# henriChevreux/distillation_trajectories

Hardware: AMD Instinct MI355X
Metric: trajectory-timesteps/sec (B×T U-Net fwd) at 16×16 T=50 (higher is better)
Workload: dtype f32 (fp32-accurate; convolutions: exact 3-plane bf16 operand split on bf16 MFMA with fp32 accumulate, or native fp32 MFMA, chosen per layer)

## Files before the change

distillation_trajectories_amd/csrc/build.py:

```python
import os
import shutil
import subprocess
import sys

HERE = os.path.dirname(os.path.abspath(__file__))
SOURCES = ["dt_conv.hip", "dt_conv_bf16.hip", "dt_conv_strip.hip", "dt_layers.hip", "dt_update.hip", "dt_metrics.hip", "dt_fused.hip", "dt_unet.hip",
           "dt_featnet.hip", "dt_inception.hip", "dt_pca.hip", "dt_fid.hip", "dt_lpips.hip", "dt_tsne.hip", "dt_quality.hip", "dt_quality_stream.hip", "dt_edit.hip", "dt_rng.hip"]
HEADERS = ["dt_internal.h", "dt_conv_forms.h", "dt_batch.h", "dt_dense64.h", "dt_quality_math.h", "dt_featnet.h", "dt_conv_epilogue.h", "dt_conv_walk.h", "dt_update_math.h", "dt_fused.h", os.path.join("..", "..", "include", "dt_hip.h"),
           os.path.join("..", "..", "include", "dt_hip_noise.h"),
           os.path.join("..", "..", "include", "dt_hip_inception.h"),
           os.path.join("..", "..", "include", "dt_hip_pca.h"),
           os.path.join("..", "..", "include", "dt_hip_fid.h"),
           os.path.join("..", "..", "include", "dt_hip_fid_cov.h"),
           os.path.join("..", "..", "include", "dt_hip_lpips.h"),
           os.path.join("..", "..", "include", "dt_hip_tsne.h"),
           os.path.join("..", "..", "include", "dt_hip_quality.h"),
           os.path.join("..", "..", "include", "dt_hip_quality_stream.h"),
           os.path.join("..", "..", "include", "dt_hip_edit.h"),
           os.path.join("..", "..", "include", "dt_hip_rng.h")]
LIB = os.path.join(HERE, "libdt_hip.so")
ARCH = "gfx950"


def hipcc_path():
    for cand in (os.environ.get("HIPCC"), "/opt/rocm/bin/hipcc", shutil.which("hipcc")):
        if cand and os.path.exists(cand):
            return cand
    raise RuntimeError("hipcc not found (looked at $HIPCC, /opt/rocm/bin/hipcc, PATH)")


OBJ_DIR = os.path.join(HERE, "_build")
# ... 113 lines not shown
```

distillation_trajectories_amd/csrc/dt_conv.hip:

```cpp
#include "dt_conv_walk.h"

namespace dt {

template <int BM, int BN>
__global__ __launch_bounds__(256, 4) void conv_gemm_kernel(const ConvParams p) {
  constexpr ConvForm F = *find_conv_form(KIND_FP32, BM, BN);
  constexpr int WN = F.wn();
  constexpr int MI = F.mi(), NI = F.ni();
  constexpr int A_PER = BM / 64, B_PER = BN / 64;
  constexpr int STAGE = (BM + BN) * 16;
  constexpr int LDS_FLOATS = 2 * STAGE > F.stage_floats() ? 2 * STAGE : F.stage_floats();
  static_assert(F.wm() == 2 && WN == 2 && MI * 64 == BM && NI * 64 == BN && LDS_FLOATS >= F.stage_floats(), "wave layout, epilogue stage");
  __shared__ __attribute__((aligned(16))) float lds[LDS_FLOATS];

  const int tid = threadIdx.x, lane = tid & 63, wave = tid >> 6;
  const int wm = wave / WN, wn = wave % WN;
  const int half = lane >> 5, l31 = lane & 31;
  const int m0 = blockIdx.x * BM, n0 = blockIdx.y * BN;
  const int HW = p.H * p.W;

  int a_off[A_PER], a_off2[A_PER], a_y[A_PER], a_x[A_PER];
  bool a_ok[A_PER];
  int a_lds[A_PER];
#pragma unroll
  for (int j = 0; j < A_PER; ++j) {
    const int q = tid + j * 256, row = q >> 2, pslot = q & 3;
    const int lslot = pslot ^ ((row >> 2) & 3);
    const int m = m0 + row;
    a_ok[j] = m < p.M;
    const int mm = a_ok[j] ? m : 0;
    const int b = mm / HW, rem = mm - b * HW;
    a_y[j] = rem / p.W;
    a_x[j] = rem - a_y[j] * p.W;
    a_off[j] = mm * p.cin_p + lslot * 4;
    a_off2[j] = mm * p.cin2_p + lslot * 4;
    a_lds[j] = q * 4;
  }
  const float *wbase = p.w + (size_t)n0 * 16 + tid * 4;

  f32x16 acc[MI][NI];
  DT_CLEAR_ACC(acc, MI, NI);

  int a_row[MI], b_row[NI];
#pragma unroll
  for (int mi = 0; mi < MI; ++mi) a_row[mi] = wm * (MI * 32) + mi * 32 + l31;
#pragma unroll
  for (int ni = 0; ni < NI; ++ni) b_row[ni] = wn * (NI * 32) + ni * 32 + l31;

  KWalk k(p);
  const int n_main = k.n_main, n_iter = k.n_iter;
  for (int it = -1; it < n_iter; ++it) {
    const bool more = it + 1 < n_iter;
    f32x4 ra[A_PER], rb[B_PER];
    if (more && it + 1 >= n_main) {
      const int c2 = it + 1 - n_main;
#pragma unroll
// ... 29 lines not shown
#pragma unroll
        for (int ni = 0; ni < NI; ++ni)
          fb[ni] = *reinterpret_cast<const f32x4 *>(B + b_row[ni] * 16 + (((2 * s + half) ^ ((b_row[ni] >> 2) & 3)) << 2));
#pragma unroll
        for (int i = 0; i < 4; ++i)
#pragma unroll
          for (int mi = 0; mi < MI; ++mi)
#pragma unroll
            for (int ni = 0; ni < NI; ++ni) {
              acc[mi][ni] = __builtin_amdgcn_mfma_f32_32x32x2f32(fa[mi][i], fb[ni][i], acc[mi][ni], 0, 0, 0);
            }
      }
    }
    if (more) {
      float *A = lds + ((it + 1) & 1) * STAGE, *B = A + BM * 16;
#pragma unroll
      for (int j = 0; j < A_PER; ++j) *reinterpret_cast<f32x4 *>(A + a_lds[j]) = ra[j];
#pragma unroll
      for (int j = 0; j < B_PER; ++j) *reinterpret_cast<f32x4 *>(B + (tid + j * 256) * 4) = rb[j];
    }
    __syncthreads();
  }

  conv_epilogue<BM, BN, 1>(p, acc, lds, m0, n0, wm, wn, half, l31);
}

int launch_splitk_epilogue(const ConvParams &p, hipStream_t s);

#define DT_GEMM_ROW(cls, kind, bm, bn, kc, wk) {{kind, bm, bn, kc, wk, cls}, conv_gemm_kernel<bm, bn>},
static const ConvKernel kGemmKernels[] = {DT_CONV_FORMS_FP32(DT_GEMM_ROW)};

int launch_conv(const ConvParams &p, hipStream_t s) {
  if (!p.in || !p.w || !p.scale || !p.shift || !p.out) return DT_E_NULL;
  if (p.cin_p % 16 || p.cout_p % 16 || p.n_p % kNPad || p.M <= 0) return DT_E_SHAPE;
  if ((long long)p.M * p.cin_p >= (1ll << 31) || (long long)p.M * p.cout_p * (p.n_dup > 1 ? p.n_dup : 1) >= (1ll << 31)) return DT_E_SHAPE;
  if (const int st = conv_admissible(p)) return st;
  {
    const double flops = 2.0 * p.M * (double)p.cout_real * ((double)p.cin_real * p.ksize * p.ksize + (p.in2 ? p.cin2_real : 0));
    ProfileScope prof(find_conv_form(p.kind, p.bm, p.bn)->cls, flops, 4.0 * p.M * ((double)p.cin_real + p.cout_real), s);
    if (p.kind == KIND_FP32) {
      conv_kernel_of(kGemmKernels, p).fn<<<dim3((p.M + p.bm - 1) / p.bm, p.n_p / p.bn, p.splits), 256, 0, s>>>(p);
      DT_LAUNCH_CHECK();
    } else if (const int st = is_strip(p.kind) ? launch_conv_strip(p, s) : launch_conv_bf16x6(p, s)) return st;
  }
  return p.splits > 1 ? launch_splitk_epilogue(p, s) : DT_OK;
}


bool conv_choice_valid(const ConvChoice &c, int slot, int n_p) {
  if (!find_conv_form(c.kind, c.bm, c.bn) || n_p % c.bn) return false;
  if (c.splits < 1 || c.splits > 9 || c.splits == 5 || c.splits == 6 || c.splits == 7) return false;
  return !c.fuse || (slot == 2 && c.splits == 1);
}

static ConvChoice heuristic_choice(int M, int n_p, int taps) {
  ConvChoice c{};
// ... 44 lines not shown

template <int S>
__device__ inline float4 splitk_finish(const ConvParams &p, unsigned m, int n, size_t slab_stride) {
  const size_t o = (size_t)m * p.cout_p + n;
  float4 a;
  if (S > 0) {
    float4 part[S > 0 ? S : 1];
#pragma unroll
    for (int z = 0; z < S; ++z) part[z] = *reinterpret_cast<const float4 *>(p.slab + z * slab_stride + o);
    a = part[0];
#pragma unroll
    for (int z = 1; z < S; ++z) { a.x += part[z].x; a.y += part[z].y; a.z += part[z].z; a.w += part[z].w; }
  } else {
    a = *reinterpret_cast<const float4 *>(p.slab + o);
    for (int z = 1; z < p.splits; ++z) {
      const float4 b = *reinterpret_cast<const float4 *>(p.slab + z * slab_stride + o);
      a.x += b.x; a.y += b.y; a.z += b.z; a.w += b.w;
    }
  }
  const float4 sc = *reinterpret_cast<const float4 *>(p.scale + n), sh = *reinterpret_cast<const float4 *>(p.shift + n);
  float4 v = make_float4(a.x * sc.x + sh.x, a.y * sc.y + sh.y, a.z * sc.z + sh.z, a.w * sc.w + sh.w);
  if (p.relu) { v.x = fmaxf(v.x, 0.f); v.y = fmaxf(v.y, 0.f); v.z = fmaxf(v.z, 0.f); v.w = fmaxf(v.w, 0.f); }
  if (p.tb) {
    const float4 t = *reinterpret_cast<const float4 *>(p.tb + (size_t)(m / (unsigned)p.m_per_tb) * p.tb_stride + n);
    v.x += t.x; v.y += t.y; v.z += t.z; v.w += t.w;
  }
  if (p.add) {
    const float4 t = *reinterpret_cast<const float4 *>(p.add + o);
    v.x += t.x; v.y += t.y; v.z += t.z; v.w += t.w;
  }
  *reinterpret_cast<float4 *>(p.out + o) = v;
  return v;
}

template <int S, bool POOL>
__global__ __launch_bounds__(256) void splitk_epilogue_kernel(const ConvParams p) {
  const unsigned c4 = (unsigned)p.cout_p >> 2;
  const size_t slab_stride = (size_t)p.M * p.cout_p;
  if (!POOL) {
    const unsigned total = (unsigned)p.M * c4;
    const bool pow2 = (c4 & (c4 - 1)) == 0;
    const int sh4 = 31 - __builtin_clz(c4);
    for (unsigned i = blockIdx.x * blockDim.x + threadIdx.x; i < total; i += gridDim.x * blockDim.x) {
      const unsigned m = pow2 ? i >> sh4 : i / c4;
      splitk_finish<S>(p, m, (int)(i - m * c4) * 4, slab_stride);
    }
  } else {
    const unsigned Wo = (unsigned)p.W >> 1, Ho = (unsigned)p.H >> 1, HW = (unsigned)(p.H * p.W);
    const unsigned total = ((unsigned)p.M >> 2) * c4;
    for (unsigned i = blockIdx.x * blockDim.x + threadIdx.x; i < total; i += gridDim.x * blockDim.x) {
      const unsigned wq = i / c4;
      const int n = (int)(i - wq * c4) * 4;
      const unsigned xo = wq % Wo, r = wq / Wo;
      const unsigned yo = r % Ho, b = r / Ho;
      const unsigned m00 = b * HW + 2 * yo * (unsigned)p.W + 2 * xo;
      const float4 a = splitk_finish<S>(p, m00, n, slab_stride), bq = splitk_finish<S>(p, m00 + 1, n, slab_stride);
      const float4 c = splitk_finish<S>(p, m00 + p.W, n, slab_stride), d = splitk_finish<S>(p, m00 + p.W + 1, n, slab_stride);
      float4 mx;
      mx.x = fmaxf(fmaxf(a.x, bq.x), fmaxf(c.x, d.x)); mx.y = fmaxf(fmaxf(a.y, bq.y), fmaxf(c.y, d.y));
      mx.z = fmaxf(fmaxf(a.z, bq.z), fmaxf(c.z, d.z)); mx.w = fmaxf(fmaxf(a.w, bq.w), fmaxf(c.w, d.w));
      *reinterpret_cast<float4 *>(p.pool_out + (size_t)wq * p.cout_p + n) = mx;
    }
  }
}

template <bool POOL>
static int launch_splitk_epilogue_t(const ConvParams &p, hipStream_t s) {
  const size_t total = (size_t)(POOL ? p.M / 4 : p.M) * (p.cout_p / 4);
  const int blocks = grid_blocks(total, 4096);
  ProfileScope prof(KC_SPLITK_EPILOGUE, 0.0, 4.0 * p.M * p.cout_p * (p.splits + 1.0 + (POOL ? 0.25 : 0.0)), s);
  switch (p.splits) {
    case 2: splitk_epilogue_kernel<2, POOL><<<blocks, 256, 0, s>>>(p); break;
    case 3: splitk_epilogue_kernel<3, POOL><<<blocks, 256, 0, s>>>(p); break;
    case 4: splitk_epilogue_kernel<4, POOL><<<blocks, 256, 0, s>>>(p); break;
    case 8: splitk_epilogue_kernel<8, POOL><<<blocks, 256, 0, s>>>(p); break;
    case 9: splitk_epilogue_kernel<9, POOL><<<blocks, 256, 0, s>>>(p); break;
    default: splitk_epilogue_kernel<0, POOL><<<blocks, 256, 0, s>>>(p); break;
  }
// ... 82 lines not shown
```

distillation_trajectories_amd/csrc/dt_conv_bf16.hip:

```cpp
#include "dt_conv_walk.h"

namespace dt {

template <int BM, int BN>
__global__ __launch_bounds__(256, BM * BN > 128 * 128 ? 2 : 3) void conv_gemm_bf16x6_kernel(const ConvParams p) {
  constexpr ConvForm F = *find_conv_form(KIND_BF16, BM, BN);
  constexpr int WM = F.wm(), WN = F.wn();
  constexpr int MI = F.mi(), NI = F.ni();
  static_assert(WM == 2 && WN == 2 && MI * 64 == BM && NI * 64 == BN, "wave layout");
  constexpr int PLANE_A = BM * 16, PLANE_B = BN * 16;
  constexpr int STAGE = 3 * (PLANE_A + PLANE_B);
  __shared__ __attribute__((aligned(16))) __bf16 lds[2 * STAGE];

  const int tid = threadIdx.x, lane = tid & 63, wave = tid >> 6;
  const int wm = wave / WN, wn = wave % WN;
  const int half = lane >> 5, l31 = lane & 31;
  const int m0 = blockIdx.x * BM, n0 = blockIdx.y * BN;
  const int HW = p.H * p.W;

  constexpr int NT = 64 * WM * WN;
  constexpr int AP = (BM * 2 + NT - 1) / NT, BP = (BN * 2 + NT - 1) / NT;
  bool a_ok[AP];
  int a_y[AP], a_x[AP], a_off[AP], a_off2[AP], a_lds[AP];
#pragma unroll
  for (int i = 0; i < AP; ++i) {
    const int item = tid + i * NT;
    const int rowi = item >> 1, hh = item & 1;
    const int m = m0 + rowi;
    a_ok[i] = item < BM * 2 && m < p.M;
    const int mm = a_ok[i] ? m : 0;
    const int b = mm / HW, rem = mm - b * HW;
    a_y[i] = rem / p.W; a_x[i] = rem - a_y[i] * p.W;
    a_off[i] = mm * p.cin_p + hh * 8;
    a_off2[i] = mm * p.cin2_p + hh * 8;
    a_lds[i] = rowi * 16 + ((hh ^ ((rowi >> 3) & 1)) << 3);
  }
  const __bf16 *wbase = reinterpret_cast<const __bf16 *>(p.w) + (size_t)n0 * 16 + tid * 8;
  const size_t w_plane = (size_t)p.n_p * 16;

  f32x16 acc[MI][NI];
  DT_CLEAR_ACC(acc, MI, NI);

  int a_frag[MI], b_frag[NI];
#pragma unroll
  for (int mi = 0; mi < MI; ++mi) {
    const int row = wm * (MI * 32) + mi * 32 + l31;
    a_frag[mi] = row * 16 + ((half ^ ((row >> 3) & 1)) << 3);
  }
#pragma unroll
  for (int ni = 0; ni < NI; ++ni) {
    const int row = wn * (NI * 32) + ni * 32 + l31;
    b_frag[ni] = row * 16 + ((half ^ ((row >> 3) & 1)) << 3);
  }

  KWalk k(p);
// ... 61 lines not shown
      }
    }
    if (more) {
      __bf16 *A = lds + ((it + 1) & 1) * STAGE, *B = A + 3 * PLANE_A;
#pragma unroll
      for (int i = 0; i < AP; ++i)
        if (tid + i * NT < BM * 2) {
          bf16x8 p1, p2, p3;
          split8(ra0[i], ra1[i], p1, p2, p3);
          *reinterpret_cast<bf16x8 *>(A + a_lds[i]) = p1;
          *reinterpret_cast<bf16x8 *>(A + PLANE_A + a_lds[i]) = p2;
          *reinterpret_cast<bf16x8 *>(A + 2 * PLANE_A + a_lds[i]) = p3;
        }
#pragma unroll
      for (int i = 0; i < BP; ++i)
        if (tid + i * NT < BN * 2) {
#pragma unroll
          for (int pl = 0; pl < 3; ++pl) *reinterpret_cast<u32x4 *>(B + pl * PLANE_B + (tid + i * NT) * 8) = rb[i][pl];
        }
    }
    __syncthreads();
  }
  static_assert(2 * STAGE * sizeof(__bf16) >= F.stage_bytes(), "epilogue stage");
  conv_epilogue<BM, BN, 1>(p, acc, reinterpret_cast<float *>(lds), m0, n0, wm, wn, half, l31);
}

#define DT_BF16_ROW(cls, kind, bm, bn, kc, wk) {{kind, bm, bn, kc, wk, cls}, conv_gemm_bf16x6_kernel<bm, bn>},
static const ConvKernel kBf16Kernels[] = {DT_CONV_FORMS_BF16(DT_BF16_ROW)};

int launch_conv_bf16x6(const ConvParams &p, hipStream_t s) {
  conv_kernel_of(kBf16Kernels, p).fn<<<dim3((p.M + p.bm - 1) / p.bm, p.n_p / p.bn, p.splits), 256, 0, s>>>(p);
  DT_LAUNCH_CHECK();
  return DT_OK;
}

__global__ void pack_conv_bf16x3_kernel(const float *__restrict__ w, __bf16 *__restrict__ wp, int cout, int cin,
                                        int ksize, int cin_p, int cin_w, int n_p, int split_c, int split_cp, size_t total) {
  for (size_t idx = blockIdx.x * (size_t)blockDim.x + threadIdx.x; idx < total; idx += (size_t)gridDim.x * blockDim.x) {
    const int pos = idx & 15;
    const size_t rowi = idx >> 4;
    const int n = rowi % n_p;
    const size_t kc = rowi / n_p;
    const int phh = pos >> 3, j = pos & 7;
    const int hh = phh ^ ((n >> 3) & 1);
    const int k = (int)kc * 16 + hh * 8 + j;
    const int tap = k / cin_w, cp = k - tap * cin_w;
    const int c = conv_real_channel(cp, cin, cin_p, split_c, split_cp);
// ... 25 lines not shown
```

distillation_trajectories_amd/csrc/dt_conv_epilogue.h:

```cpp
#pragma once
#include "dt_internal.h"

namespace dt {

typedef float f32x16 __attribute__((ext_vector_type(16)));
typedef float f32x4 __attribute__((ext_vector_type(4)));

typedef __bf16 bf16x8 __attribute__((ext_vector_type(8)));
typedef __bf16 bf16x2 __attribute__((ext_vector_type(2)));
typedef unsigned u32x4 __attribute__((ext_vector_type(4)));

__device__ inline float bf16_to_f32(__bf16 v) { return (float)v; }

__device__ inline void split8(const f32x4 lo, const f32x4 hi, bf16x8 &p1, bf16x8 &p2, bf16x8 &p3) {
#pragma unroll
  for (int i = 0; i < 8; ++i) {
    const float a = i < 4 ? lo[i] : hi[i - 4];
    const __bf16 a1 = (__bf16)a;
    const float r1 = a - (float)a1;
    const __bf16 a2 = (__bf16)r1;
    const float r2 = r1 - (float)a2;
    p1[i] = a1; p2[i] = a2; p3[i] = (__bf16)r2;
  }
}

__device__ inline void mfma_bf16x6(f32x16 &acc, const bf16x8 (&fa)[3], const bf16x8 (&fb)[3]) {
  f32x16 c = acc;
  c = __builtin_amdgcn_mfma_f32_32x32x16_bf16(fa[2], fb[0], c, 0, 0, 0);
  c = __builtin_amdgcn_mfma_f32_32x32x16_bf16(fa[1], fb[1], c, 0, 0, 0);
  c = __builtin_amdgcn_mfma_f32_32x32x16_bf16(fa[0], fb[2], c, 0, 0, 0);
  c = __builtin_amdgcn_mfma_f32_32x32x16_bf16(fa[1], fb[0], c, 0, 0, 0);
  c = __builtin_amdgcn_mfma_f32_32x32x16_bf16(fa[0], fb[1], c, 0, 0, 0);
  c = __builtin_amdgcn_mfma_f32_32x32x16_bf16(fa[0], fb[0], c, 0, 0, 0);
  acc = c;
}

template <int BM, int BN, int WK, int MI, int NI>
__device__ inline void conv_epilogue(const ConvParams &p, f32x16 (&acc)[MI][NI], float *stage, int m0, int n0, int wm, int wn,
                                     int half, int l31, int wk = 0) {
  constexpr ConvForm F = *find_conv_layout(BM, BN, WK);
  static_assert(MI == F.mi() && NI == F.ni(), "accumulator tiles of the form");
  constexpr int WM = F.wm(), P = F.pitch(), C4 = BN / 4, U = WM * C4 / 8;
  constexpr int COPY = F.copy_floats();
  const int tid = threadIdx.x;
  const int HW = p.H * p.W;
  const bool pow2 = (p.W & (p.W - 1)) == 0 && (HW & (HW - 1)) == 0;
  const int w_sh = 31 - __builtin_clz(p.W), hw_sh = 31 - __builtin_clz(HW);
  auto div_hw = [&](int m) { return pow2 ? m >> hw_sh : m / HW; };
  auto div_w = [&](int r) { return pow2 ? r >> w_sh : r / p.W; };
  const bool slab_mode = p.splits > 1;
  const size_t slab_stride = (size_t)p.M * p.cout_p;
  const int c4 = tid % C4, row0 = tid / C4;
  const int n = n0 + c4 * 4;
  const bool n_ok = n < p.cout_p;
  const int nn = n_ok ? n : 0;
  auto unit = [&](int k) __attribute__((always_inline)) {
    const float *src = stage + (row0 + k * (256 / C4)) * P + c4 * 4;
    f32x4 v = *reinterpret_cast<const f32x4 *>(src);
#pragma unroll
    for (int c = 1; c < WK; ++c) v += *reinterpret_cast<const f32x4 *>(src + c * COPY);
    return v;
  };
  auto unit_row = [&](int mi, int k) { const int row = row0 + k * (256 / C4); return m0 + (row >> 5) * (MI * 32) + mi * 32 + (row & 31); };
  auto to_stage = [&](int mi) __attribute__((always_inline)) {
    __syncthreads();
#pragma unroll
    for (int ni = 0; ni < NI; ++ni)
#pragma unroll
      for (int r = 0; r < 16; ++r) {
        const int L = 4 * half + (r & 3) + 8 * (r >> 2);
        stage[wk * COPY + (wm * 32 + L) * P + wn * (NI * 32) + ni * 32 + l31] = acc[mi][ni][r];
      }
    __syncthreads();
  };

  if (slab_mode) {
    float *slab = p.slab + (size_t)blockIdx.z * slab_stride;
#pragma unroll
    for (int mi = 0; mi < MI; ++mi) {
      to_stage(mi);
#pragma unroll
      for (int k = 0; k < U; ++k) {
        const int m = unit_row(mi, k);
        if (n_ok && m < p.M)
          *reinterpret_cast<f32x4 *>(slab + (size_t)m * p.cout_p + n) = unit(k);
      }
    }
    return;
  }

  auto pool_pass = [&](int mi, float *pool_out, const float *src, int n_src, int src_pitch, size_t out_pitch) __attribute__((always_inline)) {
    __syncthreads();
    const int Wo = p.W >> 1;
    for (int q0 = tid; q0 < n_src * WM * 8 * C4; q0 += 256) {
      const int pass = q0 / (WM * 8 * C4), q = q0 - pass * (WM * 8 * C4);
      const int pp = q / C4, qc = q % C4, j = pp & 7;
      const int yy = pow2 ? j >> (w_sh - 1) : j / Wo, xx = j - yy * Wo;
      const int L0 = 2 * yy * p.W + 2 * xx;
      const int m = m0 + (pp >> 3) * (MI * 32) + mi * 32 + L0;
      const int qn = n0 + qc * 4;
      if (m >= p.M || qn >= p.cout_p || (pass && m < p.dup_skip)) continue;
      const float *s0 = src + pass * src_pitch + ((pp >> 3) * 32 + L0) * P + qc * 4;
      const f32x4 a = *reinterpret_cast<const f32x4 *>(s0), b = *reinterpret_cast<const f32x4 *>(s0 + P);
      const f32x4 c = *reinterpret_cast<const f32x4 *>(s0 + p.W * P), d = *reinterpret_cast<const f32x4 *>(s0 + (p.W + 1) * P);
      f32x4 mx;
#pragma unroll
      for (int e = 0; e < 4; ++e) mx[e] = fmaxf(fmaxf(a[e], b[e]), fmaxf(c[e], d[e]));
      const int bimg = div_hw(m), rem = m - bimg * HW;
      const int y = div_w(rem), x = rem - y * p.W;
      *reinterpret_cast<f32x4 *>(pool_out + pass * out_pitch + (((size_t)bimg * (p.H >> 1) + (y >> 1)) * Wo + (x >> 1)) * p.cout_p + qn) = mx;
    }
  };
  f32x4 w3r[4];
#pragma unroll
  for (int e = 0; e < 4; ++e) w3r[e] = p.x3 ? *reinterpret_cast<const f32x4 *>(p.w3 + 4 * (nn + e)) : f32x4{0.f, 0.f, 0.f, 0.f};
  auto x3_skip = [&](int m, int) __attribute__((always_inline)) {
    f32x4 r;
    const int img = div_hw(m), pix = m - img * HW;
    const float *xr = p.x3 + (size_t)(img < p.x3_imgs ? img : img % p.x3_imgs) * p.x3_c * p.x3_hw + pix;
    const float x0 = xr[0], x1 = p.x3_c > 1 ? xr[p.x3_hw] : 0.f, x2 = p.x3_c > 2 ? xr[2 * p.x3_hw] : 0.f;
#pragma unroll
    for (int e = 0; e < 4; ++e) {
      const f32x4 w3 = w3r[e];
      float rs = w3[3];
      rs = fmaf(x0, w3[0], rs);
      if (p.x3_c > 1) rs = fmaf(x1, w3[1], rs);
      if (p.x3_c > 2) rs = fmaf(x2, w3[2], rs);
      r[e] = rs;
    }
    return r;
  };

#pragma unroll
  for (int mi = 0; mi < MI; ++mi) {
    f32x4 v[U];
    int mrow[U];
    bool ok[U];
    to_stage(mi);
#pragma unroll
    for (int k = 0; k < U; ++k) {
      mrow[k] = unit_row(mi, k);
      ok[k] = n_ok && mrow[k] < p.M;
    }
#pragma unroll
    for (int k = 0; k < U; ++k) v[k] = unit(k);
    if (p.n_dup) {
      const f32x4 sc = *reinterpret_cast<const f32x4 *>(p.scale + nn), sh = *reinterpret_cast<const f32x4 *>(p.shift + nn);
      f32x4 rs[U];
      int cls[U], mc[U];
#pragma unroll
      for (int k = 0; k < U; ++k) {
        mc[k] = ok[k] ? mrow[k] : m0;
        const int pix = mc[k] - div_hw(mc[k]) * HW, y = div_w(pix), x = pix - y * p.W;
        cls[k] = 3 * (y == 0 ? 0 : (y == p.H - 1 ? 2 : 1)) + (x == 0 ? 0 : (x == p.W - 1 ? 2 : 1));
      }
#pragma unroll
      for (int k = 0; k < U; ++k) rs[k] = p.x3 ? x3_skip(mc[k], nn) : f32x4{0.f, 0.f, 0.f, 0.f};
      if (p.n_dup == 2 && p.dup_stage2 && p.pool_out) {
        float *stage2 = stage + WK * COPY;
        f32x4 b0[U], b1[U];
#pragma unroll
        for (int k = 0; k < U; ++k) {
          const unsigned r0 = (unsigned)mc[k] / (unsigned)p.m_per_tb;
          const unsigned r1 = (unsigned)(p.dup_rows + (mc[k] >= p.dup_skip ? mc[k] - p.dup_skip : mc[k])) / (unsigned)p.m_per_tb;
          b0[k] = *reinterpret_cast<const f32x4 *>(p.tbc + (size_t)r0 * p.tb_stride + cls[k] * p.cout_p + nn);
          b1[k] = *reinterpret_cast<const f32x4 *>(p.tbc + (size_t)r1 * p.tb_stride + cls[k] * p.cout_p + nn);
        }
#pragma unroll
        for (int k = 0; k < U; ++k) {
          f32x4 o0 = (v[k] + b0[k]) * sc + sh, o1 = (v[k] + b1[k]) * sc + sh;
          if (p.relu) {
#pragma unroll
            for (int e = 0; e < 4; ++e) { o0[e] = fmaxf(o0[e], 0.f); o1[e] = fmaxf(o1[e], 0.f); }
          }
          o0 += rs[k]; o1 += rs[k];
          if (ok[k] && !p.skip_out) {
            *reinterpret_cast<f32x4 *>(p.out + (size_t)mrow[k] * p.cout_p + n) = o0;
            if (mrow[k] >= p.dup_skip) *reinterpret_cast<f32x4 *>(p.out + ((size_t)p.dup_rows + mrow[k] - p.dup_skip) * p.cout_p + n) = o1;
          }
          *reinterpret_cast<f32x4 *>(stage + (row0 + k * (256 / C4)) * P + c4 * 4) = o0;
          *reinterpret_cast<f32x4 *>(stage2 + (row0 + k * (256 / C4)) * P + c4 * 4) = o1;
        }
        pool_pass(mi, p.pool_out, stage, 2, WK * COPY, (size_t)((p.dup_rows - p.dup_skip) >> 2) * p.cout_p);
        continue;
      }
      for (int pass = 0; pass < p.n_dup; ++pass) {
        if (pass && m0 < p.dup_skip) break;
        f32x4 o[U];
        const int shift = pass ? pass * p.dup_rows - p.dup_skip : 0;
#pragma unroll
        for (int k = 0; k < U; ++k) {
          o[k] = f32x4{0.f, 0.f, 0.f, 0.f};
          if (ok[k]) {
            const size_t mg = (size_t)shift + mrow[k];
            const unsigned tr = (unsigned)(shift + mrow[k]) / (unsigned)p.m_per_tb;
            const f32x4 b = *reinterpret_cast<const f32x4 *>(p.tbc + (size_t)tr * p.tb_stride + cls[k] * p.cout_p + n);
            o[k] = (v[k] + b) * sc + sh;
            if (p.relu) {
#pragma unroll
              for (int e = 0; e < 4; ++e) o[k][e] = fmaxf(o[k][e], 0.f);
            }
            o[k] += rs[k];
            if (!p.skip_out) *reinterpret_cast<f32x4 *>(p.out + mg * p.cout_p + n) = o[k];
          }
        }
        if (p.pool_out) {
          if (pass) __syncthreads();
#pragma unroll
          for (int k = 0; k < U; ++k) *reinterpret_cast<f32x4 *>(stage + (row0 + k * (256 / C4)) * P + c4 * 4) = o[k];
          pool_pass(mi, p.pool_out + (size_t)(shift >> 2) * p.cout_p, stage, 1, 0, 0);
        }
      }
      continue;
    }
    if (p.in2) {
      const f32x4 b2 = *reinterpret_cast<const f32x4 *>(p.bias2 + nn);
#pragma unroll
      for (int k = 0; k < U; ++k) v[k] += b2;
    } else {
      const f32x4 sc = *reinterpret_cast<const f32x4 *>(p.scale + nn), sh = *reinterpret_cast<const f32x4 *>(p.shift + nn);
#pragma unroll
      for (int k = 0; k < U; ++k) {
        v[k] = v[k] * sc + sh;
        if (p.relu) {
#pragma unroll
          for (int e = 0; e < 4; ++e) v[k][e] = fmaxf(v[k][e], 0.f);
        }
      }
    }
    if (p.tb) {
      f32x4 t[U];
#pragma unroll
      for (int k = 0; k < U; ++k) {
        t[k] = f32x4{0.f, 0.f, 0.f, 0.f};
        if (ok[k]) t[k] = *reinterpret_cast<const f32x4 *>(p.tb + (size_t)(mrow[k] / p.m_per_tb) * p.tb_stride + n);
      }
#pragma unroll
      for (int k = 0; k < U; ++k) v[k] += t[k];
    }
    if (p.add) {
      f32x4 a[U];
#pragma unroll
      for (int k = 0; k < U; ++k) {
        a[k] = f32x4{0.f, 0.f, 0.f, 0.f};
        if (ok[k]) a[k] = *reinterpret_cast<const f32x4 *>(p.add + (size_t)mrow[k] * p.cout_p + n);
      }
#pragma unroll
      for (int k = 0; k < U; ++k) v[k] += a[k];
    }
    if (p.x3) {
#pragma unroll
      for (int k = 0; k < U; ++k)
        if (ok[k]) v[k] += x3_skip(mrow[k], nn);
    }
    if (p.head_out) {
      f32x4 hw[3];
#pragma unroll
      for (int c = 0; c < 3; ++c) {
        hw[c] = f32x4{0.f, 0.f, 0.f, 0.f};
        if (c < p.head_c && n_ok) {
#pragma unroll
          for (int e = 0; e < 4; ++e)
            if (n + e < p.head_cin) hw[c][e] = p.head_w[c * p.head_cin + n + e];
        }
      }
#pragma unroll
      for (int k = 0; k < U; ++k) {
        float part[3];
#pragma unroll
        for (int c = 0; c < 3; ++c) {
          part[c] = 0.f;
#pragma unroll
          for (int e = 0; e < 4; ++e) part[c] = fmaf(hw[c][e], v[k][e], part[c]);
#pragma unroll
          for (int off = C4 / 2; off > 0; off >>= 1) part[c] += __shfl_xor(part[c], off, 64);
        }
        if (c4 == 0 && mrow[k] < p.M) {
          f32x4 o = {part[0] + p.head_b[0], 0.f, 0.f, 0.f};
          if (p.head_c > 1) o[1] = part[1] + p.head_b[1];
          if (p.head_c > 2) o[2] = part[2] + p.head_b[2];
          *reinterpret_cast<f32x4 *>(p.head_out + (size_t)mrow[k] * 4) = o;
        }
      }
      continue;
    }
#pragma unroll
    for (int k = 0; k < U; ++k)
      if (ok[k]) *reinterpret_cast<f32x4 *>(p.out + (size_t)mrow[k] * p.cout_p + n) = v[k];
    if (p.pool_out) {
#pragma unroll
      for (int k = 0; k < U; ++k) *reinterpret_cast<f32x4 *>(stage + (row0 + k * (256 / C4)) * P + c4 * 4) = v[k];
      pool_pass(mi, p.pool_out, stage, 1, 0, 0);
    }
  }
}

template <int MI, int NI>
__device__ inline void conv_midpoint(const ConvParams &p, f32x16 (&acc)[MI][NI], int n0, int wn, int l31) {
#pragma unroll
  for (int ni = 0; ni < NI; ++ni) {
    const int n = n0 + wn * (NI * 32) + ni * 32 + l31;
    const float sc = p.scale[n], sh = p.shift[n];
#pragma unroll
    for (int mi = 0; mi < MI; ++mi)
#pragma unroll
      for (int r = 0; r < 16; ++r) {
        const float v = acc[mi][ni][r] * sc + sh;
        acc[mi][ni][r] = p.relu ? fmaxf(v, 0.f) : v;
      }
  }
}

}
```

distillation_trajectories_amd/csrc/dt_conv_strip.hip:

```cpp
#include <mutex>
#include <type_traits>

#include "dt_conv_epilogue.h"

namespace dt {

extern __shared__ __attribute__((aligned(16))) __bf16 strip_lds[];

template <int BM, int BN, int KC, int WK>
__global__ __launch_bounds__(256, find_strip_form(BM, BN, KC, WK)->waves_per_simd()) void conv_strip_bf16x6_kernel(const ConvParams p) {
  constexpr ConvForm F = *find_strip_form(BM, BN, KC, WK);
  constexpr int WN = F.wn(), WM = F.wm(), NT = 256;
  constexpr int MI = F.mi(), NI = F.ni();
  constexpr int KW = F.kw();
  static_assert(WM * WN * WK * 64 == NT && KC % WK == 0 && MI * 32 * WM == BM && NI * 32 * WN == BN && (WK == 1 || (MI == 2 && NI == 2)), "wave layout");
  constexpr int PLANE_B = F.plane_b(), STAGE_B = 3 * PLANE_B;
  constexpr int AP = F.ap();
  static_assert(2 * (BM + 2 * (F.max_w() + 1)) <= AP * NT, "strip staging reach");
  const int halo = strip_halo(p.W, BM);
  const int R = F.strip_rows(halo);
  const int RZ = F.zero_row(R);
  const int PLANE_A = F.plane_a(RZ);
  __bf16 *As = strip_lds;
  __bf16 *Bs = strip_lds + F.strip_elems(PLANE_A);
// ... 19 lines not shown
    const int mm = s_ok[i] ? m : 0;
    s_off[i] = mm * p.cin_p + hh * 8;
    s_off2[i] = mm * p.cin2_p + hh * 8;
    s_offb[i] = mm * p.b_stride + hh * 8;
    s_lds[i] = srow * 16 + ((hh ^ ((srow >> 3) & 1)) << 3);
  }
  constexpr bool B_ALL = WK > 1 && BN * 4 == NT;
  constexpr int NB = B_ALL ? KC * 3 / 2 : KC * 3, SB = B_ALL ? 2 : 1;
  static_assert(!B_ALL || (KC * 3) % 2 == 0, "weight staging");
  const bool b_thread = B_ALL || tid < BN * 2;
  const int bt = B_ALL ? (tid & (BN * 2 - 1)) : tid, bsub = B_ALL ? tid / (BN * 2) : 0;
  const size_t w_plane = (size_t)p.n_p * 16;
  const __bf16 *wbase = reinterpret_cast<const __bf16 *>(p.w) + (size_t)n0 * 16 + bt * 8 + bsub * w_plane;
  const __bf16 *wbase2 = reinterpret_cast<const __bf16 *>(p.w2) + (size_t)n0 * 16 + bt * 8 + bsub * w_plane;
  const int b_lds = bsub * PLANE_B + bt * 8;

  int a_row[MI];
  unsigned a_mask[MI];
#pragma unroll
  for (int mi = 0; mi < MI; ++mi) {
    const int row_i = wm * (MI * 32) + mi * 32 + l31;
    const int m = m0 + row_i;
    a_row[mi] = row_i + halo;
    unsigned mask = 0;
    if (m < p.M) {
      const int rem = m % HW;
      const int y = rem / p.W, x = rem - y * p.W;
#pragma unroll
      for (int t = 0; t < 9; ++t) {
        const int yy = y + t / 3 - 1, xx = x + t % 3 - 1;
        if (yy >= 0 && yy < p.H && xx >= 0 && xx < p.W) mask |= 1u << t;
      }
    }
    a_mask[mi] = mask;
  }
  int b_frag[NI];
#pragma unroll
  for (int ni = 0; ni < NI; ++ni) {
    const int row = wn * (NI * 32) + ni * 32 + l31;
    b_frag[ni] = row * 16 + ((half ^ ((row >> 3) & 1)) << 3);
  }

  f32x16 acc[MI][NI];
#pragma unroll
  for (int mi = 0; mi < MI; ++mi)
#pragma unroll
    for (int ni = 0; ni < NI; ++ni)
#pragma unroll
      for (int r = 0; r < 16; ++r) acc[mi][ni][r] = 0.f;

  const int n_main = (CC + p.splits * KC - 1) / (p.splits * KC);
  const int cc0 = blockIdx.z * n_main * KC;
  const int CC2 = p.cin2_p >> 4;
  const int n_chunks = n_main + (p.in2 ? (CC2 + KC - 1) / KC : 0);

// ... 252 lines not shown
      if (DB) load_bd(ADV_SKIP0); else load_b(ADV_SKIP0);
      if (DIRECT) {
        load_a(ga0, 0);
        if (n_skip > 1) load_a(ga1, 1);
      } else {
        load_strip(n_main);
        if (tid < 48 * KC) *reinterpret_cast<u32x4 *>(As + (tid >> 4) * PLANE_A + RZ * 16 + (tid & 15) * 8) = u32x4{0u, 0u, 0u, 0u};
        write_strip();
      }
      if (!DB) write_b(step & 1);
      __syncthreads();
    }
  }
  __builtin_amdgcn_s_setprio(0);
  if (DIRECT) {
    for (int s2 = 0; s2 < n_skip; s2 += 2) {
      skip_step(ga0, s2);
      if (s2 + 1 < n_skip) skip_step(ga1, s2 + 1);
    }
  } else {
    for (int ch = n_main; ch < n_chunks; ++ch)
      do_step(std::integral_constant<int, 4>{}, ch, true, true, ch + 1 < n_chunks, ADV_SKIP);
  }
  conv_epilogue<BM, BN, WK>(p, acc, reinterpret_cast<float *>(strip_lds), m0, n0, wm, wn, half, l31, wk);
}

#define DT_STRIP_ROW(cls, kind, bm, bn, kc, wk) {{kind, bm, bn, kc, wk, cls}, conv_strip_bf16x6_kernel<bm, bn, kc, wk>},
static const ConvKernel kStripKernels[] = {DT_CONV_FORMS_ALL_STRIP(DT_STRIP_ROW)};

static int strip_lds_attribute() {
  constexpr int kMaxDevices = 64;
  static std::mutex mu;
  static int status[kMaxDevices];
  int dev = 0;
  DT_HIP_TRY(hipGetDevice(&dev));
  if (dev < 0 || dev >= kMaxDevices) return DT_E_ARG;
  std::lock_guard<std::mutex> lock(mu);
  if (status[dev] == 0) {
    status[dev] = 1;
    for (const ConvKernel &k : kStripKernels) {
      if (!k.form.needs_lds_attribute()) continue;
      const hipError_t e = hipFuncSetAttribute(reinterpret_cast<const void *>(k.fn), hipFuncAttributeMaxDynamicSharedMemorySize, (int)k.form.lds_limit());
      if (e != hipSuccess) status[dev] = -(int)e;
    }
  }
  return status[dev] == 1 ? DT_OK : -status[dev];
}
// ... 15 lines not shown
```

distillation_trajectories_amd/csrc/dt_internal.h:

```cpp
#pragma once
#include <hip/hip_runtime.h>
#include <stddef.h>
#include <stdint.h>

#include "../../include/dt_hip.h"
#include "dt_conv_forms.h"

#define DT_HIP_TRY(expr)                         \
  do {                                           \
    hipError_t _e = (expr);                      \
    if (_e != hipSuccess) return (int)_e;        \
  } while (0)
#define DT_LAUNCH_CHECK()                        \
  do {                                           \
    hipError_t _e = hipGetLastError();           \
    if (_e != hipSuccess) return (int)_e;        \
  } while (0)

namespace dt {

enum KernelClass {
  KC_SPLITK_EPILOGUE = KC_CONV_COUNT, KC_FIRST_CONV, KC_POOL, KC_UPCAT, KC_HEAD, KC_HEAD_UP, KC_TIME_BIAS, KC_UPDATE, KC_METRICS,
  KC_WASSERSTEIN, KC_RESAMPLE, KC_FUSED, KC_PAIR_METRICS,
  KC_COUNT
};
struct ProfileScope {
  ProfileScope(int cls, double flops, double bytes, hipStream_t s);
  ~ProfileScope();
  int slot;
// ... 44 lines not shown
  int splits;
  float *slab;
  int bm, bn;
  int kind;
  const float *x3;
  const float *w3;
  int x3_hw, x3_imgs, x3_c;
  const float *in2;
  const float *w2;
  const float *bias2;
  int cin2_p, cin2_real;
  float *pool_out;
  const float *in_b, *in2_b;
  int cc_a, b_stride;
  const float *head_w, *head_b;
  float *head_out;
  int head_c, head_cin;
  const float *tbc;
  int n_dup, dup_rows;
  int dup_skip;
  int skip_out;
  int dup_stage2;
  int ccw, ccw2;
};

int launch_conv(const ConvParams &p, hipStream_t s);
int launch_conv_bf16x6(const ConvParams &p, hipStream_t s);
int launch_conv_strip(const ConvParams &p, hipStream_t s);
struct ConvKernel { ConvForm form; void (*fn)(ConvParams); };
template <size_t N>
inline const ConvKernel &conv_kernel_of(const ConvKernel (&table)[N], const ConvParams &p) {
  for (const ConvKernel &k : table)
    if (k.form.kind == p.kind && k.form.bm == p.bm && k.form.bn == p.bn) return k;
  return table[0];
}
int launch_pack_conv_bf16x3(const float *w_oihw, void *wp, int cout, int cin, int ksize, int cin_p, int cin_w, int n_p,
                            int split_c, int split_cp, hipStream_t s);
constexpr int kSplitMaxRows = 32768;

struct ConvChoice { int bm, bn, splits, kind, fuse; };
struct ConvLayer {
  int M, W;
  int n_p, cin_p;
  int taps;
  bool splittable;
  bool foldable;
// ... 51 lines not shown
```

Baseline: 358,700.

## Precompute magic-number row divisors and read epilogue params lazily from kernarg

```diff
diff --git a/distillation_trajectories_amd/csrc/build.py b/distillation_trajectories_amd/csrc/build.py
--- a/distillation_trajectories_amd/csrc/build.py
+++ b/distillation_trajectories_amd/csrc/build.py
@@ -6,7 +6,7 @@
 HERE = os.path.dirname(os.path.abspath(__file__))
 SOURCES = ["dt_conv.hip", "dt_conv_bf16.hip", "dt_conv_strip.hip", "dt_layers.hip", "dt_update.hip", "dt_metrics.hip", "dt_fused.hip", "dt_unet.hip",
            "dt_featnet.hip", "dt_inception.hip", "dt_pca.hip", "dt_fid.hip", "dt_lpips.hip", "dt_tsne.hip", "dt_quality.hip", "dt_quality_stream.hip", "dt_edit.hip", "dt_rng.hip"]
-HEADERS = ["dt_internal.h", "dt_conv_forms.h", "dt_batch.h", "dt_dense64.h", "dt_quality_math.h", "dt_featnet.h", "dt_conv_epilogue.h", "dt_conv_walk.h", "dt_update_math.h", "dt_fused.h", os.path.join("..", "..", "include", "dt_hip.h"),
+HEADERS = ["dt_internal.h", "dt_conv_forms.h", "dt_conv_rows.h", "dt_batch.h", "dt_dense64.h", "dt_quality_math.h", "dt_featnet.h", "dt_conv_epilogue.h", "dt_conv_walk.h", "dt_update_math.h", "dt_fused.h", os.path.join("..", "..", "include", "dt_hip.h"),
            os.path.join("..", "..", "include", "dt_hip_noise.h"),
            os.path.join("..", "..", "include", "dt_hip_inception.h"),
            os.path.join("..", "..", "include", "dt_hip_pca.h"),
diff --git a/distillation_trajectories_amd/csrc/dt_conv.hip b/distillation_trajectories_amd/csrc/dt_conv.hip
--- a/distillation_trajectories_amd/csrc/dt_conv.hip
+++ b/distillation_trajectories_amd/csrc/dt_conv.hip
@@ -18,6 +18,7 @@
   const int half = lane >> 5, l31 = lane & 31;
   const int m0 = blockIdx.x * BM, n0 = blockIdx.y * BN;
   const int HW = p.H * p.W;
+  const ConvRowMath rm = kernarg_row_math();
 
   int a_off[A_PER], a_off2[A_PER], a_y[A_PER], a_x[A_PER];
   bool a_ok[A_PER];
@@ -29,9 +30,9 @@
     const int m = m0 + row;
     a_ok[j] = m < p.M;
     const int mm = a_ok[j] ? m : 0;
-    const int b = mm / HW, rem = mm - b * HW;
-    a_y[j] = rem / p.W;
-    a_x[j] = rem - a_y[j] * p.W;
+    const RowPixel px = row_pixel(mm, HW, p.W, rm);
+    a_y[j] = px.y;
+    a_x[j] = px.x;
     a_off[j] = mm * p.cin_p + lslot * 4;
     a_off2[j] = mm * p.cin2_p + lslot * 4;
     a_lds[j] = q * 4;
@@ -107,7 +108,7 @@
     __syncthreads();
   }
 
-  conv_epilogue<BM, BN, 1>(p, acc, lds, m0, n0, wm, wn, half, l31);
+  conv_epilogue<BM, BN, 1, false, true>(p, acc, lds, m0, n0, wm, wn, half, l31);
 }
 
 int launch_splitk_epilogue(const ConvParams &p, hipStream_t s);
@@ -115,8 +116,11 @@
 #define DT_GEMM_ROW(cls, kind, bm, bn, kc, wk) {{kind, bm, bn, kc, wk, cls}, conv_gemm_kernel<bm, bn>},
 static const ConvKernel kGemmKernels[] = {DT_CONV_FORMS_FP32(DT_GEMM_ROW)};
 
-int launch_conv(const ConvParams &p, hipStream_t s) {
+int launch_conv(const ConvParams &p_in, hipStream_t s) {
+  ConvParams p = p_in;
   if (!p.in || !p.w || !p.scale || !p.shift || !p.out) return DT_E_NULL;
+  if (p.H < 1 || p.W < 1) return DT_E_SHAPE;
+  p.rm = make_row_math(p.H, p.W, p.m_per_tb, p.x3_imgs);
   if (p.cin_p % 16 || p.cout_p % 16 || p.n_p % kNPad || p.M <= 0) return DT_E_SHAPE;
   if ((long long)p.M * p.cin_p >= (1ll << 31) || (long long)p.M * p.cout_p * (p.n_dup > 1 ? p.n_dup : 1) >= (1ll << 31)) return DT_E_SHAPE;
   if (const int st = conv_admissible(p)) return st;
@@ -207,7 +211,7 @@
   float4 v = make_float4(a.x * sc.x + sh.x, a.y * sc.y + sh.y, a.z * sc.z + sh.z, a.w * sc.w + sh.w);
   if (p.relu) { v.x = fmaxf(v.x, 0.f); v.y = fmaxf(v.y, 0.f); v.z = fmaxf(v.z, 0.f); v.w = fmaxf(v.w, 0.f); }
   if (p.tb) {
-    const float4 t = *reinterpret_cast<const float4 *>(p.tb + (size_t)(m / (unsigned)p.m_per_tb) * p.tb_stride + n);
+    const float4 t = *reinterpret_cast<const float4 *>(p.tb + (size_t)row_tb((int)m, p.rm) * p.tb_stride + n);
     v.x += t.x; v.y += t.y; v.z += t.z; v.w += t.w;
   }
   if (p.add) {
@@ -222,23 +226,20 @@
 __global__ __launch_bounds__(256) void splitk_epilogue_kernel(const ConvParams p) {
   const unsigned c4 = (unsigned)p.cout_p >> 2;
   const size_t slab_stride = (size_t)p.M * p.cout_p;
+  const bool pow2 = (c4 & (c4 - 1)) == 0;
+  const int sh4 = 31 - __builtin_clz(c4);
   if (!POOL) {
     const unsigned total = (unsigned)p.M * c4;
-    const bool pow2 = (c4 & (c4 - 1)) == 0;
-    const int sh4 = 31 - __builtin_clz(c4);
     for (unsigned i = blockIdx.x * blockDim.x + threadIdx.x; i < total; i += gridDim.x * blockDim.x) {
       const unsigned m = pow2 ? i >> sh4 : i / c4;
       splitk_finish<S>(p, m, (int)(i - m * c4) * 4, slab_stride);
     }
   } else {
-    const unsigned Wo = (unsigned)p.W >> 1, Ho = (unsigned)p.H >> 1, HW = (unsigned)(p.H * p.W);
     const unsigned total = ((unsigned)p.M >> 2) * c4;
     for (unsigned i = blockIdx.x * blockDim.x + threadIdx.x; i < total; i += gridDim.x * blockDim.x) {
-      const unsigned wq = i / c4;
+      const unsigned wq = pow2 ? i >> sh4 : i / c4;
       const int n = (int)(i - wq * c4) * 4;
-      const unsigned xo = wq % Wo, r = wq / Wo;
-      const unsigned yo = r % Ho, b = r / Ho;
-      const unsigned m00 = b * HW + 2 * yo * (unsigned)p.W + 2 * xo;
+      const unsigned m00 = (unsigned)pool_first_row((int)wq, p.H, p.W, p.rm);
       const float4 a = splitk_finish<S>(p, m00, n, slab_stride), bq = splitk_finish<S>(p, m00 + 1, n, slab_stride);
       const float4 c = splitk_finish<S>(p, m00 + p.W, n, slab_stride), d = splitk_finish<S>(p, m00 + p.W + 1, n, slab_stride);
       float4 mx;
diff --git a/distillation_trajectories_amd/csrc/dt_conv_bf16.hip b/distillation_trajectories_amd/csrc/dt_conv_bf16.hip
--- a/distillation_trajectories_amd/csrc/dt_conv_bf16.hip
+++ b/distillation_trajectories_amd/csrc/dt_conv_bf16.hip
@@ -17,6 +17,7 @@
   const int half = lane >> 5, l31 = lane & 31;
   const int m0 = blockIdx.x * BM, n0 = blockIdx.y * BN;
   const int HW = p.H * p.W;
+  const ConvRowMath rm = kernarg_row_math();
 
   constexpr int NT = 64 * WM * WN;
   constexpr int AP = (BM * 2 + NT - 1) / NT, BP = (BN * 2 + NT - 1) / NT;
@@ -29,8 +30,8 @@
     const int m = m0 + rowi;
     a_ok[i] = item < BM * 2 && m < p.M;
     const int mm = a_ok[i] ? m : 0;
-    const int b = mm / HW, rem = mm - b * HW;
-    a_y[i] = rem / p.W; a_x[i] = rem - a_y[i] * p.W;
+    const RowPixel px = row_pixel(mm, HW, p.W, rm);
+    a_y[i] = px.y; a_x[i] = px.x;
     a_off[i] = mm * p.cin_p + hh * 8;
     a_off2[i] = mm * p.cin2_p + hh * 8;
     a_lds[i] = rowi * 16 + ((hh ^ ((rowi >> 3) & 1)) << 3);
@@ -138,7 +139,7 @@
     __syncthreads();
   }
   static_assert(2 * STAGE * sizeof(__bf16) >= F.stage_bytes(), "epilogue stage");
-  conv_epilogue<BM, BN, 1>(p, acc, reinterpret_cast<float *>(lds), m0, n0, wm, wn, half, l31);
+  conv_epilogue<BM, BN, 1, true>(p, acc, reinterpret_cast<float *>(lds), m0, n0, wm, wn, half, l31);
 }
 
 #define DT_BF16_ROW(cls, kind, bm, bn, kc, wk) {{kind, bm, bn, kc, wk, cls}, conv_gemm_bf16x6_kernel<bm, bn>},
diff --git a/distillation_trajectories_amd/csrc/dt_conv_epilogue.h b/distillation_trajectories_amd/csrc/dt_conv_epilogue.h
--- a/distillation_trajectories_amd/csrc/dt_conv_epilogue.h
+++ b/distillation_trajectories_amd/csrc/dt_conv_epilogue.h
@@ -35,19 +35,32 @@
   acc = c;
 }
 
-template <int BM, int BN, int WK, int MI, int NI>
-__device__ inline void conv_epilogue(const ConvParams &p, f32x16 (&acc)[MI][NI], float *stage, int m0, int n0, int wm, int wn,
-                                     int half, int l31, int wk = 0) {
+typedef const __attribute__((address_space(4))) ConvParams KernargConvParams;
+__device__ inline KernargConvParams &kernarg_params() {
+  typedef const __attribute__((address_space(4))) char *kernarg_ptr;
+  kernarg_ptr ka = (kernarg_ptr)__builtin_amdgcn_kernarg_segment_ptr();
+  asm volatile("" : "+s"(ka));
+  return *(KernargConvParams *)ka;
+}
+
+__device__ inline ConvRowMath kernarg_row_math() {
+#if defined(__HIP_DEVICE_COMPILE__)
+  return kernarg_params().rm;
+#else
+  return ConvRowMath{};
+#endif
+}
+
+template <int BM, int BN, int WK, bool TIGHT, class Params, int MI, int NI>
+__device__ inline void conv_epilogue_on(const Params &p, f32x16 (&acc)[MI][NI], float *stage, int m0, int n0, int wm, int wn,
+                                        int half, int l31, int wk) {
   constexpr ConvForm F = *find_conv_layout(BM, BN, WK);
   static_assert(MI == F.mi() && NI == F.ni(), "accumulator tiles of the form");
   constexpr int WM = F.wm(), P = F.pitch(), C4 = BN / 4, U = WM * C4 / 8;
   constexpr int COPY = F.copy_floats();
   const int tid = threadIdx.x;
   const int HW = p.H * p.W;
-  const bool pow2 = (p.W & (p.W - 1)) == 0 && (HW & (HW - 1)) == 0;
-  const int w_sh = 31 - __builtin_clz(p.W), hw_sh = 31 - __builtin_clz(HW);
-  auto div_hw = [&](int m) { return pow2 ? m >> hw_sh : m / HW; };
-  auto div_w = [&](int r) { return pow2 ? r >> w_sh : r / p.W; };
+  const ConvRowMath rm = kernarg_row_math();
   const bool slab_mode = p.splits > 1;
   const size_t slab_stride = (size_t)p.M * p.cout_p;
   const int c4 = tid % C4, row0 = tid / C4;
@@ -91,12 +104,10 @@
 
   auto pool_pass = [&](int mi, float *pool_out, const float *src, int n_src, int src_pitch, size_t out_pitch) __attribute__((always_inline)) {
     __syncthreads();
-    const int Wo = p.W >> 1;
     for (int q0 = tid; q0 < n_src * WM * 8 * C4; q0 += 256) {
       const int pass = q0 / (WM * 8 * C4), q = q0 - pass * (WM * 8 * C4);
       const int pp = q / C4, qc = q % C4, j = pp & 7;
-      const int yy = pow2 ? j >> (w_sh - 1) : j / Wo, xx = j - yy * Wo;
-      const int L0 = 2 * yy * p.W + 2 * xx;
+      const int L0 = pool_window(j, p.W, rm);
       const int m = m0 + (pp >> 3) * (MI * 32) + mi * 32 + L0;
       const int qn = n0 + qc * 4;
       if (m >= p.M || qn >= p.cout_p || (pass && m < p.dup_skip)) continue;
@@ -106,18 +117,23 @@
       f32x4 mx;
 #pragma unroll
       for (int e = 0; e < 4; ++e) mx[e] = fmaxf(fmaxf(a[e], b[e]), fmaxf(c[e], d[e]));
-      const int bimg = div_hw(m), rem = m - bimg * HW;
-      const int y = div_w(rem), x = rem - y * p.W;
-      *reinterpret_cast<f32x4 *>(pool_out + pass * out_pitch + (((size_t)bimg * (p.H >> 1) + (y >> 1)) * Wo + (x >> 1)) * p.cout_p + qn) = mx;
+      *reinterpret_cast<f32x4 *>(pool_out + pass * out_pitch + (size_t)pool_row(row_pixel(m, HW, p.W, rm), p.H, p.W) * p.cout_p + qn) = mx;
     }
   };
   f32x4 w3r[4];
-#pragma unroll
-  for (int e = 0; e < 4; ++e) w3r[e] = p.x3 ? *reinterpret_cast<const f32x4 *>(p.w3 + 4 * (nn + e)) : f32x4{0.f, 0.f, 0.f, 0.f};
+  auto load_w3 = [&]() __attribute__((always_inline)) {
+    if (TIGHT) return;
+#pragma unroll
+    for (int e = 0; e < 4; ++e) w3r[e] = *reinterpret_cast<const f32x4 *>(p.w3 + 4 * (nn + e));
+  };
+  if (TIGHT) {
+#pragma unroll
+    for (int e = 0; e < 4; ++e) w3r[e] = p.x3 ? *reinterpret_cast<const f32x4 *>(p.w3 + 4 * (nn + e)) : f32x4{0.f, 0.f, 0.f, 0.f};
+  }
   auto x3_skip = [&](int m, int) __attribute__((always_inline)) {
     f32x4 r;
-    const int img = div_hw(m), pix = m - img * HW;
-    const float *xr = p.x3 + (size_t)(img < p.x3_imgs ? img : img % p.x3_imgs) * p.x3_c * p.x3_hw + pix;
+    const int img = row_div(m, rm.hw), pix = m - img * HW;
+    const float *xr = p.x3 + (size_t)x3_image(img, p.x3_imgs, rm) * p.x3_c * p.x3_hw + pix;
     const float x0 = xr[0], x1 = p.x3_c > 1 ? xr[p.x3_hw] : 0.f, x2 = p.x3_c > 2 ? xr[2 * p.x3_hw] : 0.f;
 #pragma unroll
     for (int e = 0; e < 4; ++e) {
@@ -151,39 +167,52 @@
 #pragma unroll
       for (int k = 0; k < U; ++k) {
         mc[k] = ok[k] ? mrow[k] : m0;
-        const int pix = mc[k] - div_hw(mc[k]) * HW, y = div_w(pix), x = pix - y * p.W;
-        cls[k] = 3 * (y == 0 ? 0 : (y == p.H - 1 ? 2 : 1)) + (x == 0 ? 0 : (x == p.W - 1 ? 2 : 1));
-      }
-#pragma unroll
-      for (int k = 0; k < U; ++k) rs[k] = p.x3 ? x3_skip(mc[k], nn) : f32x4{0.f, 0.f, 0.f, 0.f};
+        const RowPixel px = row_pixel(mc[k], HW, p.W, rm);
+        cls[k] = pixel_class(px.y, px.x, p.H, p.W);
+      }
+#pragma unroll
+      for (int k = 0; k < U; ++k) rs[k] = f32x4{0.f, 0.f, 0.f, 0.f};
+      if (p.x3) load_w3();
+      auto skip_units = [&](int k0, int k1) __attribute__((always_inline)) {
+        if (p.x3) {
+#pragma unroll
+          for (int k = k0; k < k1; ++k) rs[k] = x3_skip(mc[k], nn);
+        }
+      };
+      if (!TIGHT) skip_units(0, U);
       if (p.n_dup == 2 && p.dup_stage2 && p.pool_out) {
         float *stage2 = stage + WK * COPY;
-        f32x4 b0[U], b1[U];
-#pragma unroll
-        for (int k = 0; k < U; ++k) {
-          const unsigned r0 = (unsigned)mc[k] / (unsigned)p.m_per_tb;
-          const unsigned r1 = (unsigned)(p.dup_rows + (mc[k] >= p.dup_skip ? mc[k] - p.dup_skip : mc[k])) / (unsigned)p.m_per_tb;
-          b0[k] = *reinterpret_cast<const f32x4 *>(p.tbc + (size_t)r0 * p.tb_stride + cls[k] * p.cout_p + nn);
-          b1[k] = *reinterpret_cast<const f32x4 *>(p.tbc + (size_t)r1 * p.tb_stride + cls[k] * p.cout_p + nn);
-        }
-#pragma unroll
-        for (int k = 0; k < U; ++k) {
-          f32x4 o0 = (v[k] + b0[k]) * sc + sh, o1 = (v[k] + b1[k]) * sc + sh;
-          if (p.relu) {
-#pragma unroll
-            for (int e = 0; e < 4; ++e) { o0[e] = fmaxf(o0[e], 0.f); o1[e] = fmaxf(o1[e], 0.f); }
+        constexpr int G = TIGHT ? (U < 2 ? U : 2) : (U < 4 ? U : 4);
+#pragma unroll
+        for (int k0 = 0; k0 < U; k0 += G) {
+          f32x4 b0[U], b1[U];
+          if (TIGHT) skip_units(k0, k0 + G);
+#pragma unroll
+          for (int k = k0; k < k0 + G; ++k) {
+            const int r0 = row_tb(mc[k], rm), r1 = row_tb(row_dup1(mc[k], p.dup_rows, p.dup_skip), rm);
+            b0[k] = *reinterpret_cast<const f32x4 *>(p.tbc + (size_t)r0 * p.tb_stride + cls[k] * p.cout_p + nn);
+            b1[k] = *reinterpret_cast<const f32x4 *>(p.tbc + (size_t)r1 * p.tb_stride + cls[k] * p.cout_p + nn);
           }
-          o0 += rs[k]; o1 += rs[k];
-          if (ok[k] && !p.skip_out) {
-            *reinterpret_cast<f32x4 *>(p.out + (size_t)mrow[k] * p.cout_p + n) = o0;
-            if (mrow[k] >= p.dup_skip) *reinterpret_cast<f32x4 *>(p.out + ((size_t)p.dup_rows + mrow[k] - p.dup_skip) * p.cout_p + n) = o1;
+#pragma unroll
+          for (int k = k0; k < k0 + G; ++k) {
+            f32x4 o0 = (v[k] + b0[k]) * sc + sh, o1 = (v[k] + b1[k]) * sc + sh;
+            if (p.relu) {
+#pragma unroll
+              for (int e = 0; e < 4; ++e) { o0[e] = fmaxf(o0[e], 0.f); o1[e] = fmaxf(o1[e], 0.f); }
+            }
+            o0 += rs[k]; o1 += rs[k];
+            if (ok[k] && !p.skip_out) {
+              *reinterpret_cast<f32x4 *>(p.out + (size_t)mrow[k] * p.cout_p + n) = o0;
+              if (mrow[k] >= p.dup_skip) *reinterpret_cast<f32x4 *>(p.out + ((size_t)p.dup_rows + mrow[k] - p.dup_skip) * p.cout_p + n) = o1;
+            }
+            *reinterpret_cast<f32x4 *>(stage + (row0 + k * (256 / C4)) * P + c4 * 4) = o0;
+            *reinterpret_cast<f32x4 *>(stage2 + (row0 + k * (256 / C4)) * P + c4 * 4) = o1;
           }
-          *reinterpret_cast<f32x4 *>(stage + (row0 + k * (256 / C4)) * P + c4 * 4) = o0;
-          *reinterpret_cast<f32x4 *>(stage2 + (row0 + k * (256 / C4)) * P + c4 * 4) = o1;
         }
         pool_pass(mi, p.pool_out, stage, 2, WK * COPY, (size_t)((p.dup_rows - p.dup_skip) >> 2) * p.cout_p);
         continue;
       }
+      if (TIGHT) skip_units(0, U);
       for (int pass = 0; pass < p.n_dup; ++pass) {
         if (pass && m0 < p.dup_skip) break;
         f32x4 o[U];
@@ -193,7 +222,7 @@
           o[k] = f32x4{0.f, 0.f, 0.f, 0.f};
           if (ok[k]) {
             const size_t mg = (size_t)shift + mrow[k];
-            const unsigned tr = (unsigned)(shift + mrow[k]) / (unsigned)p.m_per_tb;
+            const int tr = row_tb(shift + mrow[k], rm);
             const f32x4 b = *reinterpret_cast<const f32x4 *>(p.tbc + (size_t)tr * p.tb_stride + cls[k] * p.cout_p + n);
             o[k] = (v[k] + b) * sc + sh;
             if (p.relu) {
@@ -233,7 +262,7 @@
 #pragma unroll
       for (int k = 0; k < U; ++k) {
         t[k] = f32x4{0.f, 0.f, 0.f, 0.f};
-        if (ok[k]) t[k] = *reinterpret_cast<const f32x4 *>(p.tb + (size_t)(mrow[k] / p.m_per_tb) * p.tb_stride + n);
+        if (ok[k]) t[k] = *reinterpret_cast<const f32x4 *>(p.tb + (size_t)row_tb(mrow[k], rm) * p.tb_stride + n);
       }
 #pragma unroll
       for (int k = 0; k < U; ++k) v[k] += t[k];
@@ -249,6 +278,7 @@
       for (int k = 0; k < U; ++k) v[k] += a[k];
     }
     if (p.x3) {
+      load_w3();
 #pragma unroll
       for (int k = 0; k < U; ++k)
         if (ok[k]) v[k] += x3_skip(mrow[k], nn);
@@ -295,6 +325,13 @@
   }
 }
 
+template <int BM, int BN, int WK, bool LATE, bool TIGHT = false, int MI, int NI>
+__device__ inline void conv_epilogue(const ConvParams &p, f32x16 (&acc)[MI][NI], float *stage, int m0, int n0, int wm, int wn,
+                                     int half, int l31, int wk = 0) {
+  if constexpr (LATE) conv_epilogue_on<BM, BN, WK, TIGHT>(kernarg_params(), acc, stage, m0, n0, wm, wn, half, l31, wk);
+  else conv_epilogue_on<BM, BN, WK, TIGHT>(p, acc, stage, m0, n0, wm, wn, half, l31, wk);
+}
+
 template <int MI, int NI>
 __device__ inline void conv_midpoint(const ConvParams &p, f32x16 (&acc)[MI][NI], int n0, int wn, int l31) {
 #pragma unroll
diff --git a/distillation_trajectories_amd/csrc/dt_conv_rows.h b/distillation_trajectories_amd/csrc/dt_conv_rows.h
--- /dev/null
+++ b/distillation_trajectories_amd/csrc/dt_conv_rows.h
@@ -0,0 +1,69 @@
+#pragma once
+
+namespace dt {
+
+struct RowDiv {
+  unsigned mul;
+  int shift;
+};
+constexpr RowDiv make_row_div(int d) {
+  if (d < 1) d = 1;
+  int s = 0;
+  while ((1ll << s) < d) ++s;
+  return RowDiv{(unsigned)((1ull << (31 + s)) / (unsigned)d + 1ull), s};
+}
+constexpr int row_div(int n, RowDiv r) {
+  return (int)((unsigned)(((unsigned long long)((unsigned)n << 1) * r.mul) >> 32) >> r.shift);
+}
+
+struct ConvRowMath {
+  RowDiv tb;
+  RowDiv hw;
+  RowDiv w;
+  RowDiv wo;
+  RowDiv ho;
+  RowDiv x3;
+};
+constexpr ConvRowMath make_row_math(int H, int W, int m_per_tb, int x3_imgs) {
+  return ConvRowMath{make_row_div(m_per_tb), make_row_div(H * W), make_row_div(W), make_row_div(W >> 1), make_row_div(H >> 1),
+                     make_row_div(x3_imgs)};
+}
+
+struct RowPixel {
+  int img, pix, y, x;
+};
+constexpr RowPixel row_pixel(int m, int HW, int W, const ConvRowMath &r) {
+  const int img = row_div(m, r.hw), pix = m - img * HW;
+  const int y = row_div(pix, r.w);
+  return RowPixel{img, pix, y, pix - y * W};
+}
+
+constexpr int row_tb(int m, const ConvRowMath &r) { return row_div(m, r.tb); }
+constexpr int row_dup1(int m, int dup_rows, int dup_skip) { return dup_rows + (m >= dup_skip ? m - dup_skip : m); }
+
+constexpr int pixel_class(int y, int x, int H, int W) {
+  return 3 * (y == 0 ? 0 : (y == H - 1 ? 2 : 1)) + (x == 0 ? 0 : (x == W - 1 ? 2 : 1));
+}
+constexpr unsigned pixel_tap_mask(int y, int x, int H, int W) {
+  unsigned mask = 0;
+  for (int t = 0; t < 9; ++t) {
+    const int yy = y + t / 3 - 1, xx = x + t % 3 - 1;
+    if (yy >= 0 && yy < H && xx >= 0 && xx < W) mask |= 1u << t;
+  }
+  return mask;
+}
+
+constexpr int pool_window(int j, int W, const ConvRowMath &r) {
+  const int yy = row_div(j, r.wo);
+  return 2 * yy * W + 2 * (j - yy * (W >> 1));
+}
+constexpr int pool_row(const RowPixel &q, int H, int W) { return (q.img * (H >> 1) + (q.y >> 1)) * (W >> 1) + (q.x >> 1); }
+constexpr int pool_first_row(int wq, int H, int W, const ConvRowMath &r) {
+  const int rr = row_div(wq, r.wo), xo = wq - rr * (W >> 1);
+  const int b = row_div(rr, r.ho), yo = rr - b * (H >> 1);
+  return b * (H * W) + 2 * yo * W + 2 * xo;
+}
+
+constexpr int x3_image(int img, int x3_imgs, const ConvRowMath &r) { return img - row_div(img, r.x3) * x3_imgs; }
+
+}
diff --git a/distillation_trajectories_amd/csrc/dt_conv_strip.hip b/distillation_trajectories_amd/csrc/dt_conv_strip.hip
--- a/distillation_trajectories_amd/csrc/dt_conv_strip.hip
+++ b/distillation_trajectories_amd/csrc/dt_conv_strip.hip
@@ -65,15 +65,11 @@
     const int row_i = wm * (MI * 32) + mi * 32 + l31;
     const int m = m0 + row_i;
     a_row[mi] = row_i + halo;
+    const ConvRowMath rm = kernarg_row_math();
     unsigned mask = 0;
     if (m < p.M) {
-      const int rem = m % HW;
-      const int y = rem / p.W, x = rem - y * p.W;
-#pragma unroll
-      for (int t = 0; t < 9; ++t) {
-        const int yy = y + t / 3 - 1, xx = x + t % 3 - 1;
-        if (yy >= 0 && yy < p.H && xx >= 0 && xx < p.W) mask |= 1u << t;
-      }
+      const RowPixel px = row_pixel(m, HW, p.W, rm);
+      mask = pixel_tap_mask(px.y, px.x, p.H, p.W);
     }
     a_mask[mi] = mask;
   }
@@ -372,7 +368,7 @@
     for (int ch = n_main; ch < n_chunks; ++ch)
       do_step(std::integral_constant<int, 4>{}, ch, true, true, ch + 1 < n_chunks, ADV_SKIP);
   }
-  conv_epilogue<BM, BN, WK>(p, acc, reinterpret_cast<float *>(strip_lds), m0, n0, wm, wn, half, l31, wk);
+  conv_epilogue<BM, BN, WK, WK == 1>(p, acc, reinterpret_cast<float *>(strip_lds), m0, n0, wm, wn, half, l31, wk);
 }
 
 #define DT_STRIP_ROW(cls, kind, bm, bn, kc, wk) {{kind, bm, bn, kc, wk, cls}, conv_strip_bf16x6_kernel<bm, bn, kc, wk>},
diff --git a/distillation_trajectories_amd/csrc/dt_internal.h b/distillation_trajectories_amd/csrc/dt_internal.h
--- a/distillation_trajectories_amd/csrc/dt_internal.h
+++ b/distillation_trajectories_amd/csrc/dt_internal.h
@@ -5,6 +5,7 @@
 
 #include "../../include/dt_hip.h"
 #include "dt_conv_forms.h"
+#include "dt_conv_rows.h"
 
 #define DT_HIP_TRY(expr)                         \
   do {                                           \
@@ -95,6 +96,7 @@
   int skip_out;
   int dup_stage2;
   int ccw, ccw2;
+  ConvRowMath rm;
 };
 
 int launch_conv(const ConvParams &p, hipStream_t s);
```

Result: faster. 364,200 (median of 6 runs) (+1.5%).
